# MIT-SPARK/Khronos

Hardware: AMD Instinct MI355X
Metric: active-window frames/sec (+ Mvoxel-updates/sec) at 1280x720 RGB-D+labels, 2 cm voxels (higher is better)
Workload: dtype f32

## Files before the change

### khronos_amd/csrc/khr_kernels_fusion.h

```cpp
#pragma once
#include "khr_device.h"

namespace khr {


constexpr int kTile = 16;
constexpr int kMaxTick = 8;

__device__ inline void ingestTile(const float* __restrict__ depth_in, const uint8_t* __restrict__ rgb_in,
                                  const int32_t* __restrict__ label_in, float* __restrict__ depth, float* __restrict__ range,
                                  uint32_t* __restrict__ rgba, int32_t* __restrict__ label, int32_t* __restrict__ dyn,
                                  float* __restrict__ tile_max, int tile, int tw, int W, int H, float fx, float fy, float cx,
                                  float cy, int range_mode, float* d_out, float* r_out) {
  const int tx = tile % tw, ty = tile / tw;
  const int u = tx * kTile + (threadIdx.x & 15), v = ty * kTile + (threadIdx.x >> 4);
  float r = 0.f, d = 0.f;
  if (u < W && v < H) {
    const int i = v * W + u;
    d = depth_in[i];
    if (d > 0.f && isfinite(d)) {
      if (range_mode == 0) {
        r = d;
      } else {
        const float x = (static_cast<float>(u) - cx) / fx, y = (static_cast<float>(v) - cy) / fy;
// ... 138 lines not shown
  const uint32_t i = blockIdx.x * blockDim.x + threadIdx.x;
  if (i >= n) return;
  const uint32_t c = rgba[i];
  rgb[3 * i] = static_cast<uint8_t>(c);
  rgb[3 * i + 1] = static_cast<uint8_t>(c >> 8);
  rgb[3 * i + 2] = static_cast<uint8_t>(c >> 16);
}

__global__ __launch_bounds__(256) void k_vertex_map(DevFrame f, float* __restrict__ vertex) {
  const int i = blockIdx.x * blockDim.x + threadIdx.x;
  if (i >= f.W * f.H) return;
  float o[3] = {0.f, 0.f, 0.f};
  if (f.range[i] > 0.f) {
    const float d = f.depth[i];
    const int u = i % f.W, v = i / f.W;
    const float x = ((static_cast<float>(u) - f.cx) / f.fx) * d;
    const float y = ((static_cast<float>(v) - f.cy) / f.fy) * d;
    xform(f.Rw, f.tw, x, y, d, o);
  }
  vertex[3 * i] = o[0];
  vertex[3 * i + 1] = o[1];
  vertex[3 * i + 2] = o[2];
}

__global__ __launch_bounds__(256) void k_alloc_visible(DevMap m, DevParams p, DevFrame f, DevFrustum fr,
                                                      uint32_t* __restrict__ work, uint32_t* __restrict__ new_list,
                                                      volatile uint32_t* host_seed, uint32_t seed_ticket,
                                                      uint32_t* __restrict__ list_count, int epoch) {
  if (seed_ticket && blockIdx.x == 0 && threadIdx.x == 0) publishSeedCount(m, host_seed, seed_ticket);
  const int S = 2 * fr.n_steps + 1;
  const int total = S * S * S;
  const int i = blockIdx.x * blockDim.x + threadIdx.x;
  bool visible = false;
  int bx = 0, by = 0, bz = 0;
  if (i < total) {
    const int dx = i % S - fr.n_steps, dy = (i / S) % S - fr.n_steps, dz = i / (S * S) - fr.n_steps;
    bx = fr.bc.x + dx;
    by = fr.bc.y + dy;
    bz = fr.bc.z + dz;
    const bool in = blockIsCandidate(p, fr, f.R, f.t, f.max_range, bx, by, bz);
    visible = in && ownerOf(bx, by, bz, p.world) == p.rank;
  }
  uint32_t slot = kInvalidSlot;
  const uint64_t key = packKey(bx, by, bz);
  if (visible) slot = htLookup(m, key);
  const bool need = visible && slot == kInvalidSlot;
  const uint32_t fidx = waveAggInc(&m.counters[C_FREE_HEAD], need);
  bool got = false;
  if (need) {
    if (fidx < m.counters[C_N_FREE]) {
      slot = m.free_slots[fidx];
      got = true;
      m.blk_index[slot] = make_int4(bx, by, bz, epoch);
      m.blk_flags[slot] = BLK_LIVE | BLK_TRACK_DIRTY | BLK_ANY_KEEP;
      m.mesh_desc[slot] = MeshDesc{0u, 0u};
      htInsertUnique(m, key, slot);
      atomicMax(&m.counters[C_MAX_SLOT], slot + 1);
    } else {
      atomicAdd(&m.counters[C_POOL_EXHAUSTED], 1u);
      slot = kInvalidSlot;
    }
  }
  const uint32_t nidx = waveAggInc(&m.counters[C_N_NEW], got);
  if (got) new_list[nidx] = slot;
  const bool emit = visible && slot != kInvalidSlot;
  const uint32_t widx = waveAggInc(list_count, emit);
  if (emit) work[widx] = slot;
  if (list_count != &m.counters[C_N_VISIBLE]) waveAggInc(&m.counters[C_N_VISIBLE], emit);
}

struct TickFrusta {
  float R[kMaxTick][9], t[kMaxTick][3], max_range[kMaxTick];
  DevFrustum fr[kMaxTick];
};
constexpr int kTickAllocThreads = 1024;
__global__ __launch_bounds__(kTickAllocThreads) void k_tick_alloc(DevMap m, DevParams p, TickFrusta tf, int ncam, int3 lo, int3 dim,
                                                   uint32_t* __restrict__ work, uint32_t list_stride,
                                                   uint32_t* __restrict__ new_list, uint32_t* __restrict__ tick_counts, int epoch) {
  const int total = dim.x * dim.y * dim.z;
  const int i = blockIdx.x * blockDim.x + threadIdx.x;
  uint32_t seen = 0u;
  int bx = 0, by = 0, bz = 0;
  if (i < total) {
    bx = lo.x + i % dim.x;
    by = lo.y + (i / dim.x) % dim.y;
    bz = lo.z + i / (dim.x * dim.y);
    if (ownerOf(bx, by, bz, p.world) == p.rank) {
      for (int k = 0; k < ncam; ++k) {
        const DevFrustum& fr = tf.fr[k];
        if (abs(bx - fr.bc.x) > fr.n_steps || abs(by - fr.bc.y) > fr.n_steps || abs(bz - fr.bc.z) > fr.n_steps) continue;
        const bool in = blockIsCandidate(p, fr, tf.R[k], tf.t[k], tf.max_range[k], bx, by, bz);
        if (in) seen |= 1u << k;
      }
    }
  }
  const bool visible = seen != 0u;
  uint32_t slot = kInvalidSlot;
  const uint64_t key = packKey(bx, by, bz);
  if (visible) slot = htLookup(m, key);
  const bool need = visible && slot == kInvalidSlot;
  const uint32_t fidx = waveAggInc(&m.counters[C_FREE_HEAD], need);
  bool got = false;
  if (need) {
    if (fidx < m.counters[C_N_FREE]) {
      slot = m.free_slots[fidx];
      got = true;
      m.blk_index[slot] = make_int4(bx, by, bz, epoch);
      m.blk_flags[slot] = BLK_LIVE | BLK_TRACK_DIRTY | BLK_ANY_KEEP;
      m.mesh_desc[slot] = MeshDesc{0u, 0u};
      htInsertUnique(m, key, slot);
      atomicMax(&m.counters[C_MAX_SLOT], slot + 1);
    } else {
      atomicAdd(&m.counters[C_POOL_EXHAUSTED], 1u);
      slot = kInvalidSlot;
    }
  }
  const uint32_t nidx = waveAggInc(&m.counters[C_N_NEW], got);
  if (got) new_list[nidx] = slot;
  if (slot == kInvalidSlot) seen = 0u;
  __shared__ uint32_t s_cnt[kMaxTick], s_base[kMaxTick];
  if (threadIdx.x < kMaxTick) s_cnt[threadIdx.x] = 0u;
  __syncthreads();
  uint32_t loff[kMaxTick];
#pragma unroll
  for (int k = 0; k < kMaxTick; ++k) {
    loff[k] = 0u;
    if (k < ncam) loff[k] = waveAggInc(&s_cnt[k], ((seen >> k) & 1u) != 0u);
  }
  __syncthreads();
  if (threadIdx.x < static_cast<uint32_t>(ncam)) {
    const uint32_t n = s_cnt[threadIdx.x];
    s_base[threadIdx.x] = n ? atomicAdd(&tick_counts[2 * threadIdx.x], n) : 0u;
  }
  if (threadIdx.x == 64) {
    uint32_t tot = 0u;
    for (int k = 0; k < ncam; ++k) tot += s_cnt[k];
    if (tot) atomicAdd(&m.counters[C_N_VISIBLE], tot);
  }
  __syncthreads();
#pragma unroll
  for (int k = 0; k < kMaxTick; ++k)
    if (k < ncam && ((seen >> k) & 1u)) work[static_cast<size_t>(k) * list_stride + s_base[k] + loff[k]] = slot;
}

__global__ void k_begin_integrate(DevMap m, int nvox, uint32_t* wg_stats) {
  if (blockIdx.x == 0) beginIntegrate(m, nvox, wg_stats);
}
__global__ void k_tick_begin(DevMap m, int nvox, uint32_t* wg_stats, uint32_t* tick_counts, uint32_t extra_calls) {
  beginIntegrate(m, nvox, wg_stats);
  if (threadIdx.x < 6 * kMaxTick) tick_counts[threadIdx.x] = 0u;
  if (threadIdx.x == 0) m.stats[S_CUM_CALLS] += extra_calls;
}

__device__ inline void cullBlocks(const DevMap& m, const DevParams& p, const DevFrame& f, const uint32_t* __restrict__ work,
                                  const uint32_t* __restrict__ n_work, FuseList out, uint32_t wpb,
                                  uint32_t* __restrict__ n_tsdf, const float* __restrict__ tile_max, int tw, int th,
                                  uint32_t bid, uint32_t nblk, uint32_t* __restrict__ item_mask = nullptr, uint32_t cam = 0u) {
  constexpr int kPerWg = 8;
  __shared__ uint4 s_blk[kPerWg];
  __shared__ uint16_t s_item[4][kPerWg * kBandSlots];
  __shared__ uint32_t s_nkeep, s_ccnt[4], s_off[4];
  const uint32_t n = *n_work;
  const uint32_t lane = threadIdx.x & 63;
  for (uint32_t base = bid * kPerWg; base < n; base += nblk * kPerWg) {
  if (threadIdx.x == 0) s_nkeep = 0;
  if (threadIdx.x < 4) s_ccnt[threadIdx.x] = 0;
  __syncthreads();
  for (uint32_t wi = base + (threadIdx.x >> 6); wi < min(n, base + kPerWg); wi += 4) {
    const uint32_t slot = work[wi];
    const int4 bi = m.blk_index[slot];
    bool keep = true;
    if (tile_max) {
      const float margin = 1e-3f;
      const float lo[3] = {static_cast<float>(bi.x) * p.bs + 0.5f * p.vs, static_cast<float>(bi.y) * p.bs + 0.5f * p.vs,
                           static_cast<float>(bi.z) * p.bs + 0.5f * p.vs};
      const float ext = p.bs - p.vs;
      float zmin = 1e30f, zmax = -1e30f, umin = 1e30f, umax = -1e30f, vmin = 1e30f, vmax = -1e30f;
      float pcs[8][3];
#pragma unroll
      for (int k = 0; k < 8; ++k) {
        xform(f.R, f.t, lo[0] + ((k & 1) ? ext : 0.f), lo[1] + ((k & 2) ? ext : 0.f), lo[2] + ((k & 4) ? ext : 0.f), pcs[k]);
        zmin = fminf(zmin, pcs[k][2]);
        zmax = fmaxf(zmax, pcs[k][2]);
      }
      if (zmax <= -margin) keep = false;
      if (zmin > f.max_range + margin) keep = false;
      if (p.range_mode == 0 && zmax < f.min_range - margin) keep = false;
      if (keep && zmin > 0.05f) {
#pragma unroll
        for (int k = 0; k < 8; ++k) {
          const float u = (pcs[k][0] * f.fx) / pcs[k][2] + f.cx, v = (pcs[k][1] * f.fy) / pcs[k][2] + f.cy;
          umin = fminf(umin, u); umax = fmaxf(umax, u);
          vmin = fminf(vmin, v); vmax = fmaxf(vmax, v);
        }
        if (umax < -1.f || vmax < -1.f || umin > static_cast<float>(f.W) || vmin > static_cast<float>(f.H)) {
          keep = false;
        } else {
          const int tx0 = max(0, (static_cast<int>(floorf(umin)) - 1) / kTile);
          const int ty0 = max(0, (static_cast<int>(floorf(vmin)) - 1) / kTile);
          const int tx1 = min(tw - 1, (static_cast<int>(ceilf(umax)) + 2) / kTile);
          const int ty1 = min(th - 1, (static_cast<int>(ceilf(vmax)) + 2) / kTile);
          if (tx1 >= tx0 && ty1 >= ty0) {
            const int nx = tx1 - tx0 + 1, nt = nx * (ty1 - ty0 + 1);
            float mr = 0.f;
            for (int t = lane; t < nt; t += 64) mr = fmaxf(mr, tile_max[(ty0 + t / nx) * tw + tx0 + t % nx]);
#pragma unroll
            for (int o = 32; o > 0; o >>= 1) mr = fmaxf(mr, __shfl_xor(mr, o));
            if (mr < zmin - p.trunc - margin) keep = false;
          }
        }
      }
    }
    if (keep) {
      uint32_t kslot = 0;
      if (lane == 0) {
        kslot = atomicAdd(&s_nkeep, 1u);
        s_blk[kslot] = make_uint4(slot, static_cast<uint32_t>(bi.x), static_cast<uint32_t>(bi.y), static_cast<uint32_t>(bi.z));
      }
      kslot = __shfl(kslot, 0);
      const uint32_t lpi = 64u / wpb, item = lane / lpi, sub = lane % lpi;
      bool ikeep = true;
      if (tile_max && (p.dbg & 256) == 0) {
        const float margin = 1e-3f;
        const int patches = (p.vps * p.vps) >> 6, rows = 64 / p.vps, zr = p.vps / (static_cast<int>(wpb) / patches);
        const int y0 = (static_cast<int>(item) % patches) * rows, z0 = (static_cast<int>(item) / patches) * zr;
        const float lo[3] = {static_cast<float>(bi.x) * p.bs + 0.5f * p.vs, static_cast<float>(bi.y) * p.bs + (static_cast<float>(y0) + 0.5f) * p.vs,
                             static_cast<float>(bi.z) * p.bs + (static_cast<float>(z0) + 0.5f) * p.vs};
        const float ex[3] = {p.bs - p.vs, static_cast<float>(rows - 1) * p.vs, static_cast<float>(zr - 1) * p.vs};
        float zmin = 1e30f, zmax = -1e30f, umin = 1e30f, umax = -1e30f, vmin = 1e30f, vmax = -1e30f;
        float pcs[8][3];
#pragma unroll
        for (int k = 0; k < 8; ++k) {
          xform(f.R, f.t, lo[0] + ((k & 1) ? ex[0] : 0.f), lo[1] + ((k & 2) ? ex[1] : 0.f), lo[2] + ((k & 4) ? ex[2] : 0.f), pcs[k]);
          zmin = fminf(zmin, pcs[k][2]);
          zmax = fmaxf(zmax, pcs[k][2]);
        }
        if (zmax <= -margin) ikeep = false;
        if (zmin > f.max_range + margin) ikeep = false;
        if (p.range_mode == 0 && zmax < f.min_range - margin) ikeep = false;
        if (ikeep && zmin > 0.05f) {
#pragma unroll
          for (int k = 0; k < 8; ++k) {
            const float iz = __builtin_amdgcn_rcpf(pcs[k][2]);
            const float u = (pcs[k][0] * f.fx) * iz + f.cx, v = (pcs[k][1] * f.fy) * iz + f.cy;
            umin = fminf(umin, u); umax = fmaxf(umax, u);
            vmin = fminf(vmin, v); vmax = fmaxf(vmax, v);
          }
          if (umax < -2.f || vmax < -2.f || umin > static_cast<float>(f.W) + 1.f || vmin > static_cast<float>(f.H) + 1.f) {
            ikeep = false;
          } else {
            const int tx0 = max(0, (static_cast<int>(floorf(umin)) - 2) / kTile);
            const int ty0 = max(0, (static_cast<int>(floorf(vmin)) - 2) / kTile);
            const int tx1 = min(tw - 1, (static_cast<int>(ceilf(umax)) + 3) / kTile);
            const int ty1 = min(th - 1, (static_cast<int>(ceilf(vmax)) + 3) / kTile);
            const int nx = tx1 - tx0 + 1, nt = nx * (ty1 - ty0 + 1);
            if (tx1 >= tx0 && ty1 >= ty0 && nt <= 16 * static_cast<int>(lpi)) {
              float m0 = 0.f, m1 = 0.f;
              int t = static_cast<int>(sub);
              for (; t + static_cast<int>(lpi) < nt; t += 2 * static_cast<int>(lpi)) {
                const int t2 = t + static_cast<int>(lpi);
                const float a = tile_max[(ty0 + t / nx) * tw + tx0 + t % nx];
                const float b = tile_max[(ty0 + t2 / nx) * tw + tx0 + t2 % nx];
                m0 = fmaxf(m0, a);
                m1 = fmaxf(m1, b);
              }
              if (t < nt) m0 = fmaxf(m0, tile_max[(ty0 + t / nx) * tw + tx0 + t % nx]);
              float mr = fmaxf(m0, m1);
              for (uint32_t o = 1; o < lpi; o <<= 1) mr = fmaxf(mr, __shfl_xor(mr, static_cast<int>(o)));
              if (mr < zmin - p.trunc - margin) ikeep = false;
            }
          }
        }
      }
      if (ikeep && sub == 0 && item_mask) {
        const size_t mi = static_cast<size_t>(slot) * wpb + item;
        const uint32_t sh = 8u * static_cast<uint32_t>(mi & 3);
        const uint32_t old = atomicOr(&item_mask[mi >> 2], (1u << cam) << sh);
        if ((old >> sh) & 0xffu) ikeep = false;
      }
      if (ikeep && sub == 0) {
        const uint32_t cls = fuseClass(m.blk_band[static_cast<size_t>(slot) * kBandSlots + item] & kItemBandMask);
        s_item[cls][atomicAdd(&s_ccnt[cls], 1u)] = static_cast<uint16_t>((kslot << 8) | item);
      }
    }
  }
  __syncthreads();
  if (threadIdx.x < 4) s_off[threadIdx.x] = s_ccnt[threadIdx.x] ? atomicAdd(&out.counts[threadIdx.x], s_ccnt[threadIdx.x]) : 0u;
  if (threadIdx.x == 0 && s_nkeep) atomicAdd(n_tsdf, s_nkeep);
  __syncthreads();
#pragma unroll
  for (uint32_t cls = 0; cls < 4; ++cls) {
    for (uint32_t i = threadIdx.x; i < s_ccnt[cls]; i += blockDim.x) {
      const uint32_t it = s_item[cls][i];
      uint4 d = s_blk[it >> 8];
      d.x |= (it & 0xffu) << 24;
      *fuseDescPtr(out, cls, s_off[cls] + i) = d;
    }
  }
  __syncthreads();
  }
}

__global__ __launch_bounds__(256) void k_cull_blocks(DevMap m, DevParams p, DevFrame f,
                                                    const uint32_t* __restrict__ work, FuseList out, uint32_t wpb,
                                                    const float* __restrict__ tile_max, int tw, int th) {
  cullBlocks(m, p, f, work, &m.counters[C_N_VISIBLE], out, wpb, &m.counters[C_N_TSDF], tile_max, tw, th, blockIdx.x, gridDim.x);
}

struct TickFrames {
  DevFrame f[kMaxTick];
  const float* tile_max[kMaxTick];
};
__global__ __launch_bounds__(256) void k_tick_cull(DevMap m, DevParams p, TickFrames t, const uint32_t* __restrict__ work,
                                                  uint32_t list_stride, uint4* __restrict__ desc, uint32_t desc_stride, uint32_t wpb,
                                                  uint32_t* __restrict__ tick_counts, int use_tiles, int tw, int th,
                                                  uint32_t* __restrict__ item_mask) {
  const int cam = blockIdx.y;
  const int lc = item_mask ? 0 : cam;
  FuseList out{desc + static_cast<size_t>(2 * lc) * desc_stride, desc + static_cast<size_t>(2 * lc + 1) * desc_stride, desc_stride,
               &tick_counts[2 * kMaxTick + 4 * lc]};
  cullBlocks(m, p, t.f[cam], work + static_cast<size_t>(cam) * list_stride, &tick_counts[2 * cam], out, wpb, &tick_counts[2 * cam + 1],
             use_tiles ? t.tile_max[cam] : nullptr, tw, th, blockIdx.x, gridDim.x, item_mask, static_cast<uint32_t>(cam));
}

__global__ __launch_bounds__(256) void k_alloc_list(DevMap m, const int* __restrict__ idx, int n,
                                                   uint32_t* __restrict__ new_list) {
  const int i = blockIdx.x * blockDim.x + threadIdx.x;
  bool need = false;
  int bx = 0, by = 0, bz = 0;
  if (i < n) {
    bx = idx[3 * i];
    by = idx[3 * i + 1];
    bz = idx[3 * i + 2];
    need = htLookup(m, packKey(bx, by, bz)) == kInvalidSlot;
  }
  const uint32_t fidx = waveAggInc(&m.counters[C_FREE_HEAD], need);
  bool got = false;
  uint32_t slot = kInvalidSlot;
  if (need) {
    if (fidx < m.counters[C_N_FREE]) {
      slot = m.free_slots[fidx];
      got = true;
      m.blk_index[slot] = make_int4(bx, by, bz, 0);
      m.blk_flags[slot] = BLK_LIVE | BLK_TRACK_DIRTY | BLK_ANY_KEEP;
      m.mesh_desc[slot] = MeshDesc{0u, 0u};
      htInsertUnique(m, packKey(bx, by, bz), slot);
      atomicMax(&m.counters[C_MAX_SLOT], slot + 1);
    } else {
      atomicAdd(&m.counters[C_POOL_EXHAUSTED], 1u);
    }
  }
  const uint32_t nidx = waveAggInc(&m.counters[C_N_NEW], got);
  if (got) new_list[nidx] = slot;
}

__global__ __launch_bounds__(256) void k_list_live(DevMap m, uint32_t* __restrict__ work, uint32_t* counter,
                                                  uint32_t require_flags, FuseList out = FuseList{nullptr, nullptr, 0u, nullptr},
                                                  uint32_t wpb = 0u) {
  const uint32_t s = blockIdx.x * blockDim.x + threadIdx.x;
  bool live = false;
  if (s < m.counters[C_MAX_SLOT]) {
    const uint32_t fl = m.blk_flags[s];
    live = (fl & BLK_LIVE) && ((fl & require_flags) == require_flags);
  }
  const uint32_t idx = waveAggInc(counter, live);
  if (live) work[idx] = s;
  if (out.a) {
    const unsigned long long mask = __ballot(live);
    if (mask) {
      const uint32_t lane = laneId();
      const int leader = __ffsll(static_cast<long long>(mask)) - 1;
      uint32_t base = 0;
      if (lane == static_cast<uint32_t>(leader)) base = atomicAdd(&out.counts[3], static_cast<uint32_t>(__popcll(mask)) * wpb);
      base = __shfl(base, leader) + static_cast<uint32_t>(__popcll(mask & ((1ull << lane) - 1ull))) * wpb;
      if (live) {
        const int4 bi = m.blk_index[s];
        for (uint32_t it = 0; it < wpb; ++it)
          *fuseDescPtr(out, 3u, base + it) =
              make_uint4(s | (it << 24), static_cast<uint32_t>(bi.x), static_cast<uint32_t>(bi.y), static_cast<uint32_t>(bi.z));
      }
    }
  }
}

__device__ inline void initBlocks(const DevMap& m, const DevParams& p, const uint32_t* __restrict__ new_list, uint32_t bid,
                                  uint32_t nblk) {
  const uint32_t n = m.counters[C_N_NEW];
  const int nv = p.nvox;
  for (uint32_t b = bid; b < n; b += nblk) {
    const size_t slot = new_list[b];
    const uint4 z = make_uint4(0, 0, 0, 0);
    uint4* d4 = reinterpret_cast<uint4*>(m.dist + slot * nv);
    uint4* w4 = reinterpret_cast<uint4*>(m.weight + slot * nv);
    uint4* c4 = reinterpret_cast<uint4*>(m.color + slot * nv);
    uint4* l4 = reinterpret_cast<uint4*>(m.sem_label + slot * nv);
    for (int i = threadIdx.x; i < nv / 4; i += blockDim.x) {
      d4[i] = z;
      w4[i] = z;
      c4[i] = z;
      if (p.with_semantics) l4[i] = z;
    }
    uint4* f4 = reinterpret_cast<uint4*>(m.vflags + slot * nv);
    for (int i = threadIdx.x; i < nv / 16; i += blockDim.x) f4[i] = z;
    if (threadIdx.x < kBandSlots) m.blk_band[slot * kBandSlots + threadIdx.x] = 0;
    if (p.with_tracking) {
      uint4* o4 = reinterpret_cast<uint4*>(m.last_obs + slot * nv);
      uint4* q4 = reinterpret_cast<uint4*>(m.last_occ + slot * nv);
      for (int i = threadIdx.x; i < nv / 2; i += blockDim.x) {
        o4[i] = z;
        q4[i] = z;
      }
      uint64_t* fb = m.freebits + slot * (nv / 64);
      for (int i = threadIdx.x; i < nv / 64; i += blockDim.x) {
        fb[i] = 0ull;
        m.obs[slot * (nv / 64) + i] = make_ulonglong2(0ull, 0ull);
      }
    }
  }
}

__global__ __launch_bounds__(256) void k_init_blocks(DevMap m, DevParams p, const uint32_t* __restrict__ new_list) {
  initBlocks(m, p, new_list, blockIdx.x, gridDim.x);
}

__global__ __launch_bounds__(256) void k_init_cull(DevMap m, DevParams p, DevFrame f, const uint32_t* __restrict__ new_list,
                                                  const uint32_t* __restrict__ work, FuseList out, uint32_t wpb,
                                                  const float* __restrict__ tile_max, int tw, int th, uint32_t n_cull) {
  if (blockIdx.x < n_cull)
    cullBlocks(m, p, f, work, &m.counters[C_N_VISIBLE], out, wpb, &m.counters[C_N_TSDF], tile_max, tw, th, blockIdx.x, n_cull);
  else
    initBlocks(m, p, new_list, blockIdx.x - n_cull, gridDim.x - n_cull);
}

__device__ inline uint32_t foldItemRecords(uint32_t* __restrict__ blk_flags, uint16_t* __restrict__ blk_band, uint32_t s) {
  static_assert(kBandSlots == 32, "record row = 4 x 16 bytes");
  uint4* const row = reinterpret_cast<uint4*>(blk_band + static_cast<size_t>(s) * kBandSlots);
  uint32_t any = 0u;
  uint4 r[4];
#pragma unroll
  for (int i = 0; i < 4; ++i) {
    r[i] = row[i];
    any |= r[i].x | r[i].y | r[i].z | r[i].w;
  }
  const uint32_t tm = static_cast<uint32_t>(kItemTouched) * 0x00010001u, nm = static_cast<uint32_t>(kItemNeg) * 0x00010001u;
  uint32_t fl = blk_flags[s];
  if ((any & tm) == 0u) return fl;
  fl |= BLK_UPDATED | BLK_MESH_UPDATED | BLK_TRACKING_UPDATED | ((any & nm) ? BLK_HAS_NEG : 0u);
  blk_flags[s] = fl;
  const uint32_t keep = static_cast<uint32_t>(kItemBandMask) * 0x00010001u;
#pragma unroll
  for (int i = 0; i < 4; ++i) row[i] = make_uint4(r[i].x & keep, r[i].y & keep, r[i].z & keep, r[i].w & keep);
  return fl;
}
__global__ __launch_bounds__(256) void k_tracking_select(DevMap m, uint64_t lim_active, uint64_t lim_free, int force_full,
                                                        uint32_t* __restrict__ proc, uint32_t* __restrict__ ef_list,
                                                        uint32_t* __restrict__ cnt ,
                                                        uint32_t* __restrict__ cnt_next, uint16_t* __restrict__ fold_band) {
  const uint32_t s = blockIdx.x * blockDim.x + threadIdx.x;
  if (s == 0) { cnt_next[0] = 0u; cnt_next[1] = 0u; }
  bool need = false, touched = false, reload = false;
  if (s < m.counters[C_MAX_SLOT]) {
    const uint32_t fl = fold_band ? foldItemRecords(m.blk_flags, fold_band, s) : m.blk_flags[s];
    if (fl & BLK_LIVE) {
      touched = fl & BLK_TRACKING_UPDATED;
      need = force_full || (fl & (BLK_TRACKING_UPDATED | BLK_TRACK_DIRTY));
      reload = need;
      if (!need) {
        const ulonglong2 lim = reinterpret_cast<const ulonglong2*>(m.trk_lim)[s];
        need = !(lim_active <= lim.x && lim_free <= lim.y);
      }
    }
  }
  const uint32_t ip = waveAggInc(&cnt[0], need);
  if (need) {
    proc[ip] = s | (reload ? 0x80000000u : 0u);
    reinterpret_cast<ulonglong2*>(m.trk_lim)[s] = make_ulonglong2(~0ull, ~0ull);
    m.blk_flags[s] = m.blk_flags[s] & ~(BLK_TRACKING_UPDATED | BLK_HAS_ACTIVE | BLK_TRACK_DIRTY | BLK_ANY_KEEP);
  }
  const uint32_t ie = waveAggInc(&cnt[1], touched);
  if (touched) ef_list[ie] = s;
}

template <int VPS, int CH>
__global__ __launch_bounds__(256) void k_tracking_update(DevMap m, DevParams p, uint64_t stamp, uint64_t prev_stamp,
                                                        uint64_t lim_active, uint64_t lim_free,
                                                        const uint32_t* __restrict__ proc, const uint32_t* __restrict__ n_proc) {
  constexpr int NV = VPS * VPS * VPS;
  __shared__ uint64_t s_min[2][4];
  __shared__ uint32_t s_bits;
  const uint32_t n = *n_proc * CH;
  for (uint32_t wi = blockIdx.x; wi < n; wi += gridDim.x) {
    const uint32_t pe = proc[wi / CH];
    const uint32_t s = pe & 0x7fffffffu;
    const bool reload = (pe >> 31) != 0u;
    const int g0 = static_cast<int>(wi % CH) * (NV / 4 / CH);
    const size_t slot = s;
    const float4* __restrict__ dist4 = reinterpret_cast<const float4*>(m.dist + slot * NV);
    const ulonglong2* __restrict__ lobs2 = reinterpret_cast<const ulonglong2*>(m.last_obs + slot * NV);
    uint64_t* __restrict__ locc = m.last_occ + slot * NV;
    uint32_t* __restrict__ vfl4 = reinterpret_cast<uint32_t*>(m.vflags + slot * NV);
    uint64_t* __restrict__ fb = m.freebits + slot * (NV / 64);
    bool any_active = false, any_keep = false;
    uint64_t a_min = ~0ull, f_min = ~0ull;
    if (threadIdx.x == 0) s_bits = 0u;
    constexpr int G = NV / 4 / CH / 256 > 0 ? NV / 4 / CH / 256 : 1;
    constexpr int GEND = NV / 4 / CH;
    float4 d_[G];
    ulonglong2 oa_[G], ob_[G], ca_[G], cb_[G], ow_[G];
    uint32_t v4_[G];
    uint32_t need_[G];
#pragma unroll
    for (int q = 0; q < G; ++q) {
      const int gl = threadIdx.x + 256 * q, g = g0 + gl;
      if (gl < GEND) {
        d_[q] = reload ? dist4[g] : make_float4(0.f, 0.f, 0.f, 0.f);
        ow_[q] = m.obs[slot * (NV / 64) + (g >> 4)];
        v4_[q] = vfl4[g];
      }
    }
#pragma unroll
    for (int q = 0; q < G; ++q) {
      const int gl = threadIdx.x + 256 * q, g = g0 + gl;
      need_[q] = 0u;
      ca_[q] = make_ulonglong2(0ull, 0ull);
      cb_[q] = ca_[q];
      oa_[q] = ca_[q];
      ob_[q] = ca_[q];
      if (gl < GEND) {
        const uint32_t b4 = static_cast<uint32_t>(ow_[q].x >> ((4u * static_cast<uint32_t>(g)) & 63u)) & 0xfu;
        if ((b4 & 3u) != 3u) oa_[q] = lobs2[2 * g];
        if ((b4 & 12u) != 12u) ob_[q] = lobs2[2 * g + 1];
        const float dd[4] = {d_[q].x, d_[q].y, d_[q].z, d_[q].w};
#pragma unroll
        for (int k = 0; k < 4; ++k) {
          const uint8_t v = static_cast<uint8_t>(v4_[q] >> (8 * k));
          const bool occ_k = reload ? (dd[k] < p.occ_thr) : ((v & VOX_OCC) != 0);
          if (!occ_k && !(v & VOX_OCC) && !(v & VOX_EVER_FREE)) need_[q] |= 1u << k;
        }
        if (need_[q] & 3u) ca_[q] = reinterpret_cast<const ulonglong2*>(locc)[2 * g];
        if (need_[q] & 12u) cb_[q] = reinterpret_cast<const ulonglong2*>(locc)[2 * g + 1];
      }
    }
#pragma unroll
    for (int q = 0; q < G; ++q) {
      const int gl = threadIdx.x + 256 * q, g = g0 + gl;
      if (gl >= GEND) continue;
      const uint32_t v4 = v4_[q];
      const float dd[4] = {d_[q].x, d_[q].y, d_[q].z, d_[q].w};
      uint64_t lo[4] = {oa_[q].x, oa_[q].y, ob_[q].x, ob_[q].y};
      {
        const uint32_t b4 = static_cast<uint32_t>(ow_[q].x >> ((4u * static_cast<uint32_t>(g)) & 63u)) & 0xfu;
#pragma unroll
        for (int k = 0; k < 4; ++k)
          if ((b4 >> k) & 1u) lo[k] = ow_[q].y;
      }
      const uint64_t stored[4] = {ca_[q].x, ca_[q].y, cb_[q].x, cb_[q].y};
      uint32_t nv4 = 0, freebits4 = 0;
#pragma unroll
      for (int k = 0; k < 4; ++k) {
        const uint8_t v = static_cast<uint8_t>(v4 >> (8 * k));
        const bool was_occ = v & VOX_OCC;
        const bool occ = reload ? (dd[k] < p.occ_thr) : was_occ;
        uint64_t oc = stored[k];
        if (occ) {
          oc = stamp;
        } else if (was_occ) {
          oc = prev_stamp;
          locc[4 * g + k] = prev_stamp;
        }
        const bool was_active = v & VOX_ACTIVE;
        const bool active = lo[k] >= lim_active;
        uint8_t nv = static_cast<uint8_t>((v & ~(VOX_ACTIVE | VOX_OCC)) | (active ? VOX_ACTIVE : 0) | (occ ? VOX_OCC : 0));
        if (was_active && !active) nv |= VOX_TO_REMOVE;
        any_active |= active;
        any_keep |= !(nv & VOX_TO_REMOVE);
        if (active) a_min = lo[k] < a_min ? lo[k] : a_min;
        const bool ever = nv & VOX_EVER_FREE;
        const bool is_free = !ever && (oc < lim_free) && (lo[k] != 0ull);
        if (ever || is_free) freebits4 |= 1u << k;
        if (!occ && !ever && !is_free && lo[k] != 0ull) f_min = oc < f_min ? oc : f_min;
        nv4 |= static_cast<uint32_t>(nv) << (8 * k);
      }
      if (nv4 != v4) vfl4[g] = nv4;
      uint64_t w = static_cast<uint64_t>(freebits4) << (4 * (threadIdx.x & 15));
// ... 198 lines not shown
```

### khronos_amd/csrc/khronos_amd.hip

```cpp
#include <hip/hip_runtime.h>
#include <hip/hip_ext.h>
#include <hipcub/hipcub.hpp>

#include <algorithm>
#include <array>
#include <atomic>
#include <chrono>
#include <memory>
#include <mutex>
#include <cmath>
#include <cstdarg>
#include <cstdio>
#include <climits>
#include <cstring>
#include <cstdlib>
#include <functional>
#include <map>
#include <string>
#include <thread>
#include <tuple>
#include <unordered_map>
#include <vector>

#include "../../include/khronos_amd.h"
// ... 1120 lines not shown
  if (which == 0) s.dynw_valid = false;
  if (which == 1) {
    const int rca = auxAfterMain(c);
    if (rca) return rca;
  }
  return KHR_OK;
}

int khr_download_frame(khr_ctx* c, int slot, float* range, float* vertex_map, int32_t* dynamic_image) {
  if (!c || slot < 0 || slot >= static_cast<int>(c->slots.size()) || !c->slots[slot].valid) return fail(KHR_EINVAL, "bad slot");
  FrameSlot& s = c->slots[slot];
  const size_t n = static_cast<size_t>(s.sensor.width) * s.sensor.height;
  if (range) HIP_TRY(hipMemcpyAsync(range, s.vRange(), n * sizeof(float), hipMemcpyDeviceToHost, c->stream));
  if (dynamic_image) HIP_TRY(hipMemcpyAsync(dynamic_image, s.dyn, n * sizeof(int32_t), hipMemcpyDeviceToHost, c->stream));
  if (vertex_map) {
    DevTemp tmpv;
    KHR_TRY(tmpv.alloc(n * 3 * sizeof(float)));
    float* d_v = tmpv.as<float>();
    hipLaunchKernelGGL(k_vertex_map, dim3(gridFor(n)), dim3(256), 0, c->stream, makeDevFrame(c, s), d_v);
    HIP_TRY(hipMemcpyAsync(vertex_map, d_v, n * 3 * sizeof(float), hipMemcpyDeviceToHost, c->stream));
    HIP_TRY(hipStreamSynchronize(c->stream));
  }
  HIP_TRY(hipStreamSynchronize(c->stream));
  return KHR_OK;
}

struct khr_frame_copy {
  std::shared_ptr<khr_ctx::FramePool> pool;
  DevBuf<uint8_t> block;
  int device = 0;
  Event ready;
  DevFrame f{};
  size_t n = 0, n_pad = 0;
};

int khr_frame_copy_create(khr_ctx* c, int slot, khr_frame_copy** out) {
  if (!c || !out || slot < 0 || slot >= static_cast<int>(c->slots.size()) || !c->slots[slot].valid) return fail(KHR_EINVAL, "bad argument");
  HIP_TRY(hipSetDevice(c->device));
  FrameSlot& s = c->slots[slot];
  const size_t n = static_cast<size_t>(s.sensor.width) * s.sensor.height, n_pad = (n + 3) / 4 * 4;
  if (n_pad > c->cfg.max_frame_pixels) return fail(KHR_EINVAL, "frame larger than max_frame_pixels");
  auto fc = std::make_unique<khr_frame_copy>();
  fc->pool = c->frame_pool;
  fc->device = c->device;
  const size_t bytes = 16 * n_pad;
  {
    std::lock_guard<std::mutex> lock(c->frame_pool->mu);
    auto& fr = c->frame_pool->free;
    for (size_t i = 0; i < fr.size(); ++i)
      if (fr[i].count() >= bytes) {
        fc->block = std::move(fr[i]);
        fr.erase(fr.begin() + static_cast<long>(i));
        break;
      }
  }
  if (!fc->block && fc->block.alloc(bytes)) return fail(KHR_ENOMEM, "frame copy (%zu bytes)", bytes);
  if (fc->ready.ensure()) return fail(KHR_EDEVICE, "event");
  if (s.aux_seq) HIP_TRY(hipStreamWaitEvent(c->stream, c->ev_aux_done, 0));
  hipLaunchKernelGGL(k_frame_copy, dim3(512), dim3(256), 0, c->stream, reinterpret_cast<const uint4*>(s.vDepth()),
                     reinterpret_cast<const uint4*>(s.vRange()), s.has_color ? reinterpret_cast<const uint4*>(s.vRgba()) : nullptr,
                     s.has_label ? reinterpret_cast<const uint4*>(s.vLabel()) : nullptr, reinterpret_cast<uint4*>(fc->block.get()),
                     static_cast<uint32_t>(n_pad / 4));
  HIP_TRY(hipGetLastError());
  HIP_TRY(hipEventRecord(fc->ready, c->stream));
  fc->f = makeDevFrame(c, s);
  fc->f.depth = reinterpret_cast<const float*>(fc->block.get());
  fc->f.range = reinterpret_cast<const float*>(fc->block + 4 * n_pad);
  fc->f.rgba = reinterpret_cast<const uint32_t*>(fc->block + 8 * n_pad);
  fc->f.label = reinterpret_cast<const int32_t*>(fc->block + 12 * n_pad);
  fc->f.dyn = nullptr;
  fc->f.obj = nullptr;
  fc->n = n;
  fc->n_pad = n_pad;
  *out = fc.release();
  return KHR_OK;
}

int khr_frame_copy_download(khr_frame_copy* fc, float* depth, float* range, uint8_t* color_rgb, int32_t* labels, float* vertex_map) {
  if (!fc) return fail(KHR_EINVAL, "null frame copy");
  HIP_TRY(hipSetDevice(fc->device));
  HIP_TRY(hipEventSynchronize(fc->ready));
  const size_t n = fc->n;
  if (depth) HIP_TRY(hipMemcpy(depth, fc->f.depth, n * 4, hipMemcpyDeviceToHost));
  if (range) HIP_TRY(hipMemcpy(range, fc->f.range, n * 4, hipMemcpyDeviceToHost));
  if (labels) HIP_TRY(hipMemcpy(labels, fc->f.label, n * 4, hipMemcpyDeviceToHost));
  if (color_rgb || vertex_map) {
    DevTemp tmp;
    KHR_TRY(tmp.alloc(n * 12));
    if (color_rgb) {
      hipLaunchKernelGGL(k_rgba_to_rgb, dim3(static_cast<unsigned>((n + 255) / 256)), dim3(256), 0, nullptr, fc->f.rgba, tmp.as<uint8_t>(), static_cast<uint32_t>(n));
      HIP_TRY(hipMemcpy(color_rgb, tmp.get(), n * 3, hipMemcpyDeviceToHost));
    }
    if (vertex_map) {
      hipLaunchKernelGGL(k_vertex_map, dim3(static_cast<unsigned>((n + 255) / 256)), dim3(256), 0, nullptr, fc->f, tmp.as<float>());
      HIP_TRY(hipMemcpy(vertex_map, tmp.get(), n * 12, hipMemcpyDeviceToHost));
    }
  }
  return KHR_OK;
}

void khr_frame_copy_release(khr_frame_copy* fc) {
  if (!fc) return;
  hipSetDevice(fc->device);
  if (fc->ready) hipEventSynchronize(fc->ready);
  {
    std::lock_guard<std::mutex> lock(fc->pool->mu);
    if (!fc->pool->dead && fc->pool->free.size() < 8) fc->pool->free.push_back(std::move(fc->block));
  }
  delete fc;
}

int khr_copy_frame_image(khr_ctx* c, int slot, int which, void* device_dst) {
  if (!c || !device_dst || slot < 0 || slot >= static_cast<int>(c->slots.size()) || !c->slots[slot].valid) return fail(KHR_EINVAL, "bad argument");
  if (which != 0 && which != 1) return fail(KHR_EINVAL, "which must be 0 (dynamic) or 1 (object)");
  HIP_TRY(hipSetDevice(c->device));
  FrameSlot& s = c->slots[slot];
  const size_t n = static_cast<size_t>(s.sensor.width) * s.sensor.height;
  if (which == 1 && !s.has_obj) {
    HIP_TRY(hipMemsetAsync(device_dst, 0, n * sizeof(int32_t), c->stream));
    return KHR_OK;
  }
  if (which == 1) {
    HIP_TRY(hipEventRecord(c->ev_aux_done, c->aux_stream));
    HIP_TRY(hipStreamWaitEvent(c->stream, c->ev_aux_done, 0));
  }
  HIP_TRY(hipMemcpyAsync(device_dst, which == 0 ? s.dyn : s.obj, n * sizeof(int32_t), hipMemcpyDeviceToDevice, c->stream));
  return KHR_OK;
}

int khr_download_frame_image(khr_ctx* c, int slot, int which, int32_t* image) {
  if (!c || !image || slot < 0 || slot >= static_cast<int>(c->slots.size()) || !c->slots[slot].valid) return fail(KHR_EINVAL, "bad argument");
  if (which != 0 && which != 1) return fail(KHR_EINVAL, "which must be 0 (dynamic) or 1 (object)");
  FrameSlot& s = c->slots[slot];
  const size_t n = static_cast<size_t>(s.sensor.width) * s.sensor.height;
  if (which == 1 && !s.has_obj) {
    std::memset(image, 0, n * sizeof(int32_t));
    return KHR_OK;
  }
  if (which == 1) HIP_TRY(hipStreamSynchronize(c->aux_stream));
  HIP_TRY(hipMemcpyAsync(image, which == 0 ? s.dyn : s.obj, n * sizeof(int32_t), hipMemcpyDeviceToHost, c->stream));
  HIP_TRY(hipStreamSynchronize(c->stream));
  return KHR_OK;
}

static int integrateAlloc(khr_ctx* c, FrameSlot& s, const DevFrame& f, int allocate_blocks) {
  DevMap& m = c->m;
  if (!c->begun) hipLaunchKernelGGL(k_begin_integrate, dim3(1), dim3(256), 0, c->stream, m, c->p.nvox, c->d_wg_stats);
  c->begun = false;
  if (allocate_blocks) {
    ScopedTimer tm(c, 3);
    const DevFrustum fr = makeFrustum(c, f);
    const int S = 2 * fr.n_steps + 1;
    const size_t total = static_cast<size_t>(S) * S * S;
    hipLaunchKernelGGL(k_alloc_visible, dim3(gridFor(total)), dim3(256), 0, c->stream, m, c->p, f, fr, c->d_work, c->d_new,
                       c->h_pinned.dev() + 2, c->seed_publish_pending ? c->seed_ticket : 0u, &m.counters[C_N_VISIBLE], 0);
    c->seed_publish_pending = false;
    hipLaunchKernelGGL(k_init_cull, dim3(1024 + 1024), dim3(256), 0, c->stream, m, c->p, f, c->d_new, c->d_work,
                       FuseList{c->d_work4, c->d_work4 + c->item_cap, c->item_cap, &m.counters[C_N_ITEMS0]}, c->wpb,
                       c->cfg.disable_culling ? nullptr : s.vTileMax(), s.tw, s.th, 1024u);
    c->host_index_valid = false, ++c->map_gen;
  } else {
    hipLaunchKernelGGL(k_list_live, dim3(gridFor(m.capacity)), dim3(256), 0, c->stream, m, c->d_work,
                       &m.counters[C_N_VISIBLE], 0u, FuseList{c->d_work4, c->d_work4 + c->item_cap, c->item_cap, &m.counters[C_N_ITEMS0]},
                       c->wpb);
  }
  HIP_TRY(hipGetLastError());
  return KHR_OK;
}

struct UpdateLists {
  FuseList list{nullptr, nullptr, 0u, nullptr};
};

static int fuseGrid(khr_ctx* c, const void* kernel, int group, int block) {
  static std::map<std::pair<int, const void*>, int> cache;
  static std::mutex cache_mu;
  std::lock_guard<std::mutex> lock(cache_mu);
  const std::pair<int, const void*> key{c->device, kernel};
  auto it = cache.find(key);
  if (it != cache.end()) return it->second;
  int per_cu = 0, cus = 256;
  if (hipOccupancyMaxActiveBlocksPerMultiprocessor(&per_cu, kernel, block, 0) != hipSuccess || per_cu < 1) per_cu = 1;
  per_cu = std::min(per_cu, std::max(1, kUpdateWavesPerCu / (block / 64)));
  hipDeviceProp_t prop;
  if (hipGetDeviceProperties(&prop, c->device) == hipSuccess && prop.multiProcessorCount > 0) cus = prop.multiProcessorCount;
  per_cu = std::min(per_cu, 8);
  int grid = std::min(kUpdateStatSlots, per_cu * cus);
  grid = std::max(8 * group, grid / (8 * group) * (8 * group));
  cache[key] = grid;
  return grid;
}

static int fuse2Grid(khr_ctx* c, const void* kern, int wpw) {
  static std::map<std::pair<int, const void*>, int> cache;
  static std::mutex mu;
  std::lock_guard<std::mutex> lock(mu);
  const std::pair<int, const void*> key{c->device, kern};
  auto it = cache.find(key);
  if (it != cache.end()) return it->second;
  int per_cu = 0;
  if (hipOccupancyMaxActiveBlocksPerMultiprocessor(&per_cu, kern, 64 * wpw, 0) != hipSuccess || per_cu < 1) per_cu = 1;
  hipDeviceProp_t prop;
  int cus = 256;
  if (hipGetDeviceProperties(&prop, c->device) == hipSuccess && prop.multiProcessorCount > 0) cus = prop.multiProcessorCount;
  const int grid = std::min(kUpdateStatSlots, per_cu * cus) / 8 * 8;
  cache[key] = grid;
  return grid;
}

static void fillFuseFrame(const khr_ctx* c, const FrameSlot& s, const DevFrame& f, int use_mask, int object_id, FuseFrame* a) {
  a->range = f.range; a->dyn = f.dyn; a->rgba = f.rgba; a->label = f.label; a->obj = f.obj;
  a->W = f.W; a->H = f.H; a->fx = f.fx; a->fy = f.fy; a->cx = f.cx; a->cy = f.cy; a->min_range = f.min_range; a->max_range = f.max_range;
  std::memcpy(a->R, f.R, sizeof(a->R));
  std::memcpy(a->t, f.t, sizeof(a->t));
  a->stamp = f.stamp;
  a->use_mask = (use_mask && !s.dyn_clean) ? 1 : 0;
  a->has_color = f.has_color;
  a->object_id = object_id;
  a->do_sem = (c->p.with_semantics && ((c->p.sem_mode == 1) ? (object_id >= 0 && f.obj != nullptr) : (f.has_label != 0))) ? 1 : 0;
  a->tile_max = s.vTileMax();
  a->tw = s.tw;
  a->th = s.th;
}
static void fillFuseMap(khr_ctx* c, FuseArgs* a) {
  DevMap& m = c->m;
  a->blk_index = m.blk_index; a->blk_flags = m.blk_flags; a->dist = m.dist; a->weight = m.weight; a->last_obs = m.last_obs; a->obs = m.obs;
  a->color = m.color; a->vflags = m.vflags; a->sem_label = m.sem_label; a->lik = m.lik; a->wg_stats = c->d_wg_stats;
  a->blk_band = m.blk_band;
  a->vs = c->p.vs; a->bs = c->p.bs; a->trunc = c->p.trunc; a->dropoff_eps = c->p.dropoff_eps; a->max_weight = c->p.max_weight;
  a->adaptive_diff = c->p.adaptive_diff; a->log_match = c->p.log_match; a->log_nomatch = c->p.log_nomatch;
  a->interp = c->p.interp; a->range_mode = c->p.range_mode; a->use_dropoff = c->p.use_dropoff; a->const_weight = c->p.const_weight;
  a->with_tracking = c->p.with_tracking;
  a->K = c->p.K; a->KS = c->p.KS; a->sem_mode = c->p.sem_mode;
  a->band_mode = c->cfg.max_frame_pixels <= 640u * 480u ? 0 : 1;
  a->sink = c->d_fuse_sink;
  a->blend_pre = c->cfg.color_blend_weight != 0;
}

static int integrateUpdateMulti(khr_ctx* c, khr_ctx* src, const int* src_slots, const int* object_ids, int n_frames, int use_mask) {
  if (c->cfg.voxels_per_side != 8 || n_frames < 2 || n_frames > kMaxMultiFrames) return 1;
  FuseArgs a{};
  fillFuseMap(c, &a);
  const bool defcfg = a.range_mode == 0 && a.interp == 2 && a.use_dropoff && !a.const_weight;
  if (!defcfg) return 1;
  if (!c->h_frames) {
    if (c->h_frames.alloc(kMaxMultiFrames) || c->d_frames.alloc(kMaxMultiFrames)) return fail(KHR_ENOMEM, "frame argument staging");
    KHR_TRY(c->ev_frames.ensure());
  } else {
    HIP_TRY(hipEventSynchronize(c->ev_frames));
  }
  for (int i = 0; i < n_frames; ++i) {
    FrameSlot& s = src->slots[src_slots[i]];
    const DevFrame f = makeDevFrame(src, s);
    fillFuseFrame(c, s, f, use_mask, object_ids ? object_ids[i] : -1, &c->h_frames[i]);
  }
  {
    const uint32_t n_words = static_cast<uint32_t>(sizeof(FuseFrame) / 4) * static_cast<uint32_t>(n_frames);
    hipLaunchKernelGGL(k_copy_words, dim3((n_words + 255) / 256), dim3(256), 0, c->stream, reinterpret_cast<const uint32_t*>(c->h_frames.dev()),
                       reinterpret_cast<uint32_t*>(c->d_frames.get()), n_words);
  }
  HIP_TRY(hipEventRecord(c->ev_frames, c->stream));
  static_cast<FuseFrame&>(a) = c->h_frames[0];
  a.frames = c->d_frames;
  a.n_frames = n_frames;
  if (c->item_cap > 0) {
    const int n_words = (n_frames + 31) / 32;
    const size_t need = static_cast<size_t>(c->item_cap) * static_cast<size_t>(n_words);
    if (need > c->d_frame_bits.count()) {
      const size_t want = static_cast<size_t>(c->item_cap) * static_cast<size_t>((n_words + 3) / 4 * 4);
      HIP_TRY(hipStreamSynchronize(c->stream));
      if (c->d_frame_bits.reserve(want)) return fail(KHR_ENOMEM, "frame bits of the multi-frame update (%zu bytes)", want * sizeof(uint32_t));
    }
    const uint64_t tests = static_cast<uint64_t>(c->explicit_blocks > 0 ? std::min<uint64_t>(c->explicit_blocks, c->m.capacity) : c->m.capacity) *
                           c->wpb * static_cast<uint64_t>(n_words) * 32u;
    const unsigned grid = static_cast<unsigned>(std::min<uint64_t>((tests + 255) / 256, 8192));
    hipLaunchKernelGGL((k_multi_cull<8>), dim3(std::max(1u, grid)), dim3(256), 0, c->stream, c->m.blk_flags, c->m.blk_index, &c->m.counters[C_MAX_SLOT],
                       c->p.vs, c->p.bs, c->p.trunc, static_cast<const FuseFrame*>(c->d_frames.get()), n_frames, n_words, c->wpb, BLK_LIVE, c->d_frame_bits);
    HIP_TRY(hipGetLastError());
    a.frame_bits = c->d_frame_bits;
    a.frame_words = n_words;
  }
  FuseList list{c->d_work4, c->d_work4 + c->item_cap, c->item_cap, &c->m.counters[C_N_ITEMS0]};
  if (a.frame_bits != nullptr) {
    if (!c->d_multi_list) {
      HIP_TRY(hipStreamSynchronize(c->stream));
      if (c->d_multi_list.alloc(2 * static_cast<size_t>(c->item_cap) + 1)) return fail(KHR_ENOMEM, "item list of the multi-frame update");
    }
    uint32_t* const counts = reinterpret_cast<uint32_t*>(c->d_multi_list + 2 * static_cast<size_t>(c->item_cap));
    HIP_TRY(hipMemsetAsync(counts, 0, 16, c->stream));
    list = FuseList{c->d_multi_list, c->d_multi_list + c->item_cap, c->item_cap, counts};
    const uint64_t n_it = static_cast<uint64_t>(c->explicit_blocks > 0 ? std::min<uint64_t>(c->explicit_blocks, c->m.capacity) : c->m.capacity) * c->wpb;
    hipLaunchKernelGGL(k_multi_order, dim3(static_cast<unsigned>((n_it + 1023) / 1024)), dim3(1024), 0, c->stream, c->m.blk_flags, c->m.blk_index,
                       &c->m.counters[C_MAX_SLOT], static_cast<const uint32_t*>(c->d_frame_bits.get()), a.frame_words, n_frames, c->wpb, BLK_LIVE, list);
    HIP_TRY(hipGetLastError());
  }
  constexpr int WPW = 8;
  auto go = [&](auto kern) {
    static std::map<std::pair<int, const void*>, std::pair<int, int>> per_cu_of;
    static std::mutex per_cu_mu;
    int per_cu = 0, cus = 256;
    {
      std::lock_guard<std::mutex> lock(per_cu_mu);
      const std::pair<int, const void*> key{c->device, reinterpret_cast<const void*>(kern)};
      auto it = per_cu_of.find(key);
      if (it != per_cu_of.end()) {
        per_cu = it->second.first;
        cus = it->second.second;
      } else {
        if (hipOccupancyMaxActiveBlocksPerMultiprocessor(&per_cu, kern, 64 * WPW, 0) != hipSuccess || per_cu < 1) per_cu = 1;
        hipDeviceProp_t prop;
        if (hipGetDeviceProperties(&prop, c->device) == hipSuccess && prop.multiProcessorCount > 0) cus = prop.multiProcessorCount;
        per_cu_of[key] = {per_cu, cus};
// ... 4157 lines not shown
```

Baseline: 3954.

## Fuse block allocation, culling and init into one kernel with LDS candidate list

Replaces the separate alloc-visible kernel and the combined init/cull kernel with one 1024-thread kernel. Each workgroup tests 256 frustum candidates, allocates missing blocks, keeps survivors in an LDS list, culls them, and zeroes newly allocated blocks, so the global work and new-block lists are no longer written and re-read. Fresh blocks go straight to the full-fuse class without reading band records. In exchange the many small grid-strided kernels become fewer large workgroups, which may hurt occupancy and load balance, and block init now runs serially per workgroup.

```diff
diff --git a/khronos_amd/csrc/khr_kernels_fusion.h b/khronos_amd/csrc/khr_kernels_fusion.h
--- a/khronos_amd/csrc/khr_kernels_fusion.h
+++ b/khronos_amd/csrc/khr_kernels_fusion.h
@@ -314,23 +314,42 @@
   if (threadIdx.x == 0) m.stats[S_CUM_CALLS] += extra_calls;
 }
 
-__device__ inline void cullBlocks(const DevMap& m, const DevParams& p, const DevFrame& f, const uint32_t* __restrict__ work,
-                                  const uint32_t* __restrict__ n_work, FuseList out, uint32_t wpb,
-                                  uint32_t* __restrict__ n_tsdf, const float* __restrict__ tile_max, int tw, int th,
-                                  uint32_t bid, uint32_t nblk, uint32_t* __restrict__ item_mask = nullptr, uint32_t cam = 0u) {
-  constexpr int kPerWg = 8;
-  __shared__ uint4 s_blk[kPerWg];
-  __shared__ uint16_t s_item[4][kPerWg * kBandSlots];
+struct CullWorkList {
+  const uint32_t* __restrict__ work;
+  const int4* __restrict__ blk_index;
+  __device__ void get(uint32_t wi, uint32_t* slot, int4* bi, bool* fresh) const {
+    *slot = work[wi];
+    *bi = blk_index[*slot];
+    *fresh = false;
+  }
+};
+struct CullLdsList {
+  const uint4* list;
+  __device__ void get(uint32_t wi, uint32_t* slot, int4* bi, bool* fresh) const {
+    const uint4 e = list[wi];
+    *slot = e.x & 0x7fffffffu;
+    *bi = make_int4(static_cast<int>(e.y), static_cast<int>(e.z), static_cast<int>(e.w), 0);
+    *fresh = (e.x >> 31) != 0u;
+  }
+};
+constexpr int kCullChunk = 8;
+template <int CHUNK, int WAVES, class Src>
+__device__ inline void cullChunk(const DevMap& m, const DevParams& p, const DevFrame& f, const Src& src, uint32_t base, uint32_t n,
+                                 FuseList out, uint32_t wpb, uint32_t* __restrict__ n_tsdf, const float* __restrict__ tile_max, int tw,
+                                 int th, uint32_t* __restrict__ item_mask, uint32_t cam) {
+  static_assert(CHUNK <= 256, "an item entry is survivor << 8 | item in 16 bits");
+  __shared__ uint4 s_blk[CHUNK];
+  __shared__ uint16_t s_item[4][CHUNK * kBandSlots];
   __shared__ uint32_t s_nkeep, s_ccnt[4], s_off[4];
-  const uint32_t n = *n_work;
   const uint32_t lane = threadIdx.x & 63;
-  for (uint32_t base = bid * kPerWg; base < n; base += nblk * kPerWg) {
   if (threadIdx.x == 0) s_nkeep = 0;
   if (threadIdx.x < 4) s_ccnt[threadIdx.x] = 0;
   __syncthreads();
-  for (uint32_t wi = base + (threadIdx.x >> 6); wi < min(n, base + kPerWg); wi += 4) {
-    const uint32_t slot = work[wi];
-    const int4 bi = m.blk_index[slot];
+  for (uint32_t wi = base + (threadIdx.x >> 6); wi < min(n, base + CHUNK); wi += WAVES) {
+    uint32_t slot;
+    int4 bi;
+    bool fresh;
+    src.get(wi, &slot, &bi, &fresh);
     bool keep = true;
     if (tile_max) {
       const float margin = 1e-3f;
@@ -441,7 +460,7 @@
         if ((old >> sh) & 0xffu) ikeep = false;
       }
       if (ikeep && sub == 0) {
-        const uint32_t cls = fuseClass(m.blk_band[static_cast<size_t>(slot) * kBandSlots + item] & kItemBandMask);
+        const uint32_t cls = fresh ? 3u : fuseClass(m.blk_band[static_cast<size_t>(slot) * kBandSlots + item] & kItemBandMask);
         s_item[cls][atomicAdd(&s_ccnt[cls], 1u)] = static_cast<uint16_t>((kslot << 8) | item);
       }
     }
@@ -460,13 +479,16 @@
     }
   }
   __syncthreads();
-  }
-}
-
-__global__ __launch_bounds__(256) void k_cull_blocks(DevMap m, DevParams p, DevFrame f,
-                                                    const uint32_t* __restrict__ work, FuseList out, uint32_t wpb,
-                                                    const float* __restrict__ tile_max, int tw, int th) {
-  cullBlocks(m, p, f, work, &m.counters[C_N_VISIBLE], out, wpb, &m.counters[C_N_TSDF], tile_max, tw, th, blockIdx.x, gridDim.x);
+}
+
+__device__ inline void cullBlocks(const DevMap& m, const DevParams& p, const DevFrame& f, const uint32_t* __restrict__ work,
+                                  const uint32_t* __restrict__ n_work, FuseList out, uint32_t wpb,
+                                  uint32_t* __restrict__ n_tsdf, const float* __restrict__ tile_max, int tw, int th,
+                                  uint32_t bid, uint32_t nblk, uint32_t* __restrict__ item_mask = nullptr, uint32_t cam = 0u) {
+  const uint32_t n = *n_work;
+  const CullWorkList src{work, m.blk_index};
+  for (uint32_t base = bid * kCullChunk; base < n; base += nblk * kCullChunk)
+    cullChunk<kCullChunk, 4>(m, p, f, src, base, n, out, wpb, n_tsdf, tile_max, tw, th, item_mask, cam);
 }
 
 struct TickFrames {
@@ -545,39 +567,45 @@
   }
 }
 
+__device__ inline void initBlock(const DevMap& m, const DevParams& p, size_t slot) {
+  const int nv = p.nvox;
+  const uint4 z = make_uint4(0, 0, 0, 0);
+  uint4* d4 = reinterpret_cast<uint4*>(m.dist + slot * nv);
+  uint4* w4 = reinterpret_cast<uint4*>(m.weight + slot * nv);
+  uint4* c4 = reinterpret_cast<uint4*>(m.color + slot * nv);
+  uint4* l4 = reinterpret_cast<uint4*>(m.sem_label + slot * nv);
+  for (int i = threadIdx.x; i < nv / 4; i += blockDim.x) {
+    d4[i] = z;
+    w4[i] = z;
+    c4[i] = z;
+    if (p.with_semantics) l4[i] = z;
+  }
+  uint4* f4 = reinterpret_cast<uint4*>(m.vflags + slot * nv);
+  for (int i = threadIdx.x; i < nv / 16; i += blockDim.x) f4[i] = z;
+  if (threadIdx.x < kBandSlots) m.blk_band[slot * kBandSlots + threadIdx.x] = 0;
+  if (p.with_tracking) {
+    uint4* o4 = reinterpret_cast<uint4*>(m.last_obs + slot * nv);
+    uint4* q4 = reinterpret_cast<uint4*>(m.last_occ + slot * nv);
+    for (int i = threadIdx.x; i < nv / 2; i += blockDim.x) {
+      o4[i] = z;
+      q4[i] = z;
+    }
+    uint64_t* fb = m.freebits + slot * (nv / 64);
+    for (int i = threadIdx.x; i < nv / 64; i += blockDim.x) {
+      fb[i] = 0ull;
+      m.obs[slot * (nv / 64) + i] = make_ulonglong2(0ull, 0ull);
+    }
+  }
+}
 __device__ inline void initBlocks(const DevMap& m, const DevParams& p, const uint32_t* __restrict__ new_list, uint32_t bid,
                                   uint32_t nblk) {
   const uint32_t n = m.counters[C_N_NEW];
-  const int nv = p.nvox;
-  for (uint32_t b = bid; b < n; b += nblk) {
-    const size_t slot = new_list[b];
-    const uint4 z = make_uint4(0, 0, 0, 0);
-    uint4* d4 = reinterpret_cast<uint4*>(m.dist + slot * nv);
-    uint4* w4 = reinterpret_cast<uint4*>(m.weight + slot * nv);
-    uint4* c4 = reinterpret_cast<uint4*>(m.color + slot * nv);
-    uint4* l4 = reinterpret_cast<uint4*>(m.sem_label + slot * nv);
-    for (int i = threadIdx.x; i < nv / 4; i += blockDim.x) {
-      d4[i] = z;
-      w4[i] = z;
-      c4[i] = z;
-      if (p.with_semantics) l4[i] = z;
-    }
-    uint4* f4 = reinterpret_cast<uint4*>(m.vflags + slot * nv);
-    for (int i = threadIdx.x; i < nv / 16; i += blockDim.x) f4[i] = z;
-    if (threadIdx.x < kBandSlots) m.blk_band[slot * kBandSlots + threadIdx.x] = 0;
-    if (p.with_tracking) {
-      uint4* o4 = reinterpret_cast<uint4*>(m.last_obs + slot * nv);
-      uint4* q4 = reinterpret_cast<uint4*>(m.last_occ + slot * nv);
-      for (int i = threadIdx.x; i < nv / 2; i += blockDim.x) {
-        o4[i] = z;
-        q4[i] = z;
-      }
-      uint64_t* fb = m.freebits + slot * (nv / 64);
-      for (int i = threadIdx.x; i < nv / 64; i += blockDim.x) {
-        fb[i] = 0ull;
-        m.obs[slot * (nv / 64) + i] = make_ulonglong2(0ull, 0ull);
-      }
-    }
+  for (uint32_t b = bid; b < n; b += nblk) initBlock(m, p, new_list[b]);
+}
+__device__ inline void initLdsBlocks(const DevMap& m, const DevParams& p, const uint4* list, uint32_t n) {
+  for (uint32_t b = 0; b < n; ++b) {
+    const uint32_t e = list[b].x;
+    if (e >> 31) initBlock(m, p, e & 0x7fffffffu);
   }
 }
 
@@ -585,13 +613,67 @@
   initBlocks(m, p, new_list, blockIdx.x, gridDim.x);
 }
 
-__global__ __launch_bounds__(256) void k_init_cull(DevMap m, DevParams p, DevFrame f, const uint32_t* __restrict__ new_list,
-                                                  const uint32_t* __restrict__ work, FuseList out, uint32_t wpb,
-                                                  const float* __restrict__ tile_max, int tw, int th, uint32_t n_cull) {
-  if (blockIdx.x < n_cull)
-    cullBlocks(m, p, f, work, &m.counters[C_N_VISIBLE], out, wpb, &m.counters[C_N_TSDF], tile_max, tw, th, blockIdx.x, n_cull);
-  else
-    initBlocks(m, p, new_list, blockIdx.x - n_cull, gridDim.x - n_cull);
+constexpr int kAllocThreads = 1024;
+constexpr int kAllocCand = 256;
+constexpr int kAllocChunk = 24;
+static_assert(kAllocCand <= kAllocThreads && kAllocCand % 64 == 0, "whole waves take the candidates");
+__global__ __launch_bounds__(kAllocThreads) void k_alloc_cull_init(DevMap m, DevParams p, DevFrame f, DevFrustum fr, FuseList out, uint32_t wpb,
+                                                        const float* __restrict__ tile_max, int tw, int th,
+                                                        volatile uint32_t* host_seed, uint32_t seed_ticket) {
+  __shared__ uint4 s_list[kAllocCand];
+  __shared__ uint32_t s_n, s_nnew;
+  if (seed_ticket && blockIdx.x == 0 && threadIdx.x == 0) publishSeedCount(m, host_seed, seed_ticket);
+  if (threadIdx.x == 0) {
+    s_n = 0u;
+    s_nnew = 0u;
+  }
+  __syncthreads();
+  const int S = 2 * fr.n_steps + 1;
+  const int total = S * S * S;
+  const int i = static_cast<int>(threadIdx.x * gridDim.x + blockIdx.x);
+  bool visible = false;
+  int bx = 0, by = 0, bz = 0;
+  if (threadIdx.x < kAllocCand && i < total) {
+    const int dx = i % S - fr.n_steps, dy = (i / S) % S - fr.n_steps, dz = i / (S * S) - fr.n_steps;
+    bx = fr.bc.x + dx;
+    by = fr.bc.y + dy;
+    bz = fr.bc.z + dz;
+    const bool in = blockIsCandidate(p, fr, f.R, f.t, f.max_range, bx, by, bz);
+    visible = in && ownerOf(bx, by, bz, p.world) == p.rank;
+  }
+  uint32_t slot = kInvalidSlot;
+  const uint64_t key = packKey(bx, by, bz);
+  if (visible) slot = htLookup(m, key);
+  const bool need = visible && slot == kInvalidSlot;
+  const uint32_t fidx = waveAggInc(&m.counters[C_FREE_HEAD], need);
+  bool got = false;
+  if (need) {
+    if (fidx < m.counters[C_N_FREE]) {
+      slot = m.free_slots[fidx];
+      got = true;
+      m.blk_index[slot] = make_int4(bx, by, bz, 0);
+      m.blk_flags[slot] = BLK_LIVE | BLK_TRACK_DIRTY | BLK_ANY_KEEP;
+      m.mesh_desc[slot] = MeshDesc{0u, 0u};
+      htInsertUnique(m, key, slot);
+      atomicMax(&m.counters[C_MAX_SLOT], slot + 1);
+    } else {
+      atomicAdd(&m.counters[C_POOL_EXHAUSTED], 1u);
+      slot = kInvalidSlot;
+    }
+  }
+  const bool emit = visible && slot != kInvalidSlot;
+  const uint32_t li = waveAggInc(&s_n, emit);
+  if (emit)
+    s_list[li] = make_uint4(slot | (got ? 0x80000000u : 0u), static_cast<uint32_t>(bx), static_cast<uint32_t>(by), static_cast<uint32_t>(bz));
+  waveAggInc(&s_nnew, got);
+  __syncthreads();
+  const uint32_t n = s_n;
+  if (threadIdx.x == 0 && n) atomicAdd(&m.counters[C_N_VISIBLE], n);
+  if (threadIdx.x == 64 && s_nnew) atomicAdd(&m.counters[C_N_NEW], s_nnew);
+  const CullLdsList src{s_list};
+  for (uint32_t base = 0; base < n; base += kAllocChunk)
+    cullChunk<kAllocChunk, kAllocThreads / 64>(m, p, f, src, base, n, out, wpb, &m.counters[C_N_TSDF], tile_max, tw, th, nullptr, 0u);
+  initLdsBlocks(m, p, s_list, n);
 }
 
 __device__ inline uint32_t foldItemRecords(uint32_t* __restrict__ blk_flags, uint16_t* __restrict__ blk_band, uint32_t s) {
diff --git a/khronos_amd/csrc/khronos_amd.hip b/khronos_amd/csrc/khronos_amd.hip
--- a/khronos_amd/csrc/khronos_amd.hip
+++ b/khronos_amd/csrc/khronos_amd.hip
@@ -1296,12 +1296,11 @@
     const DevFrustum fr = makeFrustum(c, f);
     const int S = 2 * fr.n_steps + 1;
     const size_t total = static_cast<size_t>(S) * S * S;
-    hipLaunchKernelGGL(k_alloc_visible, dim3(gridFor(total)), dim3(256), 0, c->stream, m, c->p, f, fr, c->d_work, c->d_new,
-                       c->h_pinned.dev() + 2, c->seed_publish_pending ? c->seed_ticket : 0u, &m.counters[C_N_VISIBLE], 0);
+    hipLaunchKernelGGL(k_alloc_cull_init, dim3(static_cast<unsigned>((total + kAllocCand - 1) / kAllocCand)), dim3(kAllocThreads), 0, c->stream, m,
+                       c->p, f, fr, FuseList{c->d_work4, c->d_work4 + c->item_cap, c->item_cap, &m.counters[C_N_ITEMS0]}, c->wpb,
+                       c->cfg.disable_culling ? nullptr : s.vTileMax(), s.tw, s.th, c->h_pinned.dev() + 2,
+                       c->seed_publish_pending ? c->seed_ticket : 0u);
     c->seed_publish_pending = false;
-    hipLaunchKernelGGL(k_init_cull, dim3(1024 + 1024), dim3(256), 0, c->stream, m, c->p, f, c->d_new, c->d_work,
-                       FuseList{c->d_work4, c->d_work4 + c->item_cap, c->item_cap, &m.counters[C_N_ITEMS0]}, c->wpb,
-                       c->cfg.disable_culling ? nullptr : s.vTileMax(), s.tw, s.th, 1024u);
     c->host_index_valid = false, ++c->map_gen;
   } else {
     hipLaunchKernelGGL(k_list_live, dim3(gridFor(m.capacity)), dim3(256), 0, c->stream, m, c->d_work,
```

New measurement: 3944 (median of 2 runs). No clear change (-0.3%).
